# lasseufpa/intent_radio_sched_multi_slice

Hardware: AMD Instinct MI355X
Metric: env-steps/s (batched TTIs) at mult_slice 10-slice/100-UE; 1->8 GPU scaling [device-policy rollout over batch partitions; step-by-step and learner-in-the-loop schedules beside it] (higher is better)
Workload: dtype f64

## Files before the change

### intent_radio_sched_multi_slice_amd/csrc/ranenv_host.cpp

```cpp
#include <algorithm>
#include <cctype>
#include <cmath>
#include <cstdarg>
#include <cstdio>
#include <cstdlib>
#include <cstring>
#include <functional>
#include <new>
#include <string>
#include <array>
#include <vector>

#include "ranenv_internal.h"

using namespace ranenv_dev;

namespace {
thread_local std::string g_last_error;
constexpr int N_STEP_BUILDS = SB_PERSIST_TINY + 1;

}

enum NetRole { NET_INTER, NET_INTRA, NET_INTER_VALUE, NET_INTRA_VALUE, NET_HEAD_CLIP, NET_HEAD_TANH, NET_HEAD_VALUE, NET_SAC_Q };
enum NetForm { FORM_ONE, FORM_SLICE, FORM_MEMBER };
// ... 35 lines not shown
    bool slice_on = false;
    ranenv_trace trace{}; bool trace_on = false;
    std::vector<int32_t> trace_env, trace_slot;
    int32_t *d_trace = nullptr; int trace_cap = 0;
    std::vector<int32_t> sh_steps; bool sh_valid = false;
    const uint8_t *last_done = nullptr;
    int32_t *d_plist = nullptr, *d_pcount = nullptr; PersistCtl *d_pctl = nullptr; unsigned long long *d_pslots = nullptr;
    int p_nclass = 0, p_cap = 0;
    std::vector<int32_t> pcount_host; bool pclass_dirty = true, pcount_host_stale = true;
    bool pclass_maybe = false;
    int *d_cls_flag = nullptr;
    int *h_perr = nullptr;
    int *d_perr_dev = nullptr;
    int perr_seen = 0;
    int last_rollout_persistent = 0, last_rollout_launches = 0;
    long long last_rollout_lean_ttis = 0;
    uint64_t step_launches[N_STEP_BUILDS][2] = {};
    std::string launch_note;
    int p_wave_slots[2] = {0, 0};
    int n_parts = 1;
    std::vector<hipStream_t> part_stream;
    std::vector<hipEvent_t> part_done, part_in;
    std::vector<int> part_lo;
    hipEvent_t ev_in = nullptr;
    bool prof_on = false;
    std::vector<hipEvent_t> prof_ev;
    size_t prof_used = 0;
    long long prof_ttis = 0;
    long long prof_env_ttis = 0;
    struct NetSlot {
// ... 205 lines not shown
    *ev0 = h->prof_ev[h->prof_used]; *ev1 = h->prof_ev[h->prof_used + 1];
    h->prof_used += 2; h->prof_ttis += n_tti; h->prof_env_ttis += (long long)n * n_tti;
    return hipSuccess;
}

const char *const step_build_names[N_STEP_BUILDS] = {"lean", "small", "gather", "tiny1", "mixed", "packed", "persist", "persist_tiny"};

hipError_t launch_step_counted(ranenv_handle h, const StepLaunch &l, dim3 grid, dim3 block, hipStream_t s, hipEvent_t ev0, hipEvent_t ev1, const KP &kp)
{
    const hipError_t e = launch_step(l, grid, block, s, ev0, ev1, kp);
    const bool known = l.build >= 0 && l.build < N_STEP_BUILDS;
    if (e == hipSuccess) {
        if (known && (l.mode & 3) == MODE_STEP) h->step_launches[l.build][l.many ? 1 : 0]++;
        if (l.members) h->last_rollout_member_lines = 1;
        if ((l.mode & 3) == MODE_STEP && l.many && kp.lean_tail != 0 && kp.n_tti > 1) h->last_rollout_lean_ttis += kp.n_tti - 1;
    } else {
        char buf[160];
        snprintf(buf, sizeof(buf), "step kernel build '%s' (row width %d, mode %d, %s, %s): %s", known ? step_build_names[l.build] : "?", l.np, l.mode,
                 l.many ? "several TTIs" : "one TTI", l.gather ? "gather" : "stream", hipGetErrorString(e));
        h->launch_note = buf;
    }
    return e;
}

struct StepFacts { int mode, n_tti, compact; bool gather; int e0, n; bool lines = false, masked = false, tiles = false; };
struct StepChoice { StepLaunch l; dim3 grid, block; int compact; };
StepChoice step_choice(const ranenv *h, const StepFacts &f)
{
    const bool step = f.mode == MODE_STEP;
    const bool pe = f.mode != MODE_RESET && scale_per_element(h);
    const bool many = step && f.n_tti > 1;
    const bool mixed = step && !pe && h->mix != 0 && f.compact != 0 && h->nt == 2 * WAVE && f.e0 == 0 && f.n == h->cfg.batch && !f.masked &&
                       (h->mix == 2 || !persist_tiny(h)) && RANENV_DIAG == 0;
    const int compact = f.compact != 0 && (mixed || f.gather || f.compact == 2) ? 1 : 0;
    const dim3 grid((unsigned)f.n), block((unsigned)h->nt);
    if (mixed) return {{h->np, SB_MIXED, MODE_STEP, many, f.gather}, grid, dim3(2 * WAVE), compact};
    if (step && !pe && h->pack && h->np == 8 && h->cfg.n_ues <= 32 && h->nt == WAVE && (f.n & 1) == 0 && !f.masked && pack_fits_32(h))
        return {{8, SB_PACKED, MODE_STEP, many, f.gather}, dim3((unsigned)(f.n / 2)), dim3(WAVE), compact};
    StepLaunch l{h->np, SB_LEAN, pe ? f.mode | MODE_PE : f.mode, many, f.gather};
    if (f.gather) l.build = SB_GATHER;
    else if (!pe && step && !many && h->tiny_step && persist_tiny(h)) l.build = SB_TINY1;
    else if (!pe && h->small_batch) l.build = SB_SMALL;
    l.members = l.build == SB_LEAN && many && !pe && f.lines && compact != 0 && !f.tiles;
    return {l, grid, block, compact};
}
StepLaunch persist_choice(const ranenv *h, bool lines, bool plain = false)
{
    const bool gather = h->se_mode == RANENV_SE_GATHER, tiny = !gather && !plain && persist_tiny(h);
// ... 489 lines not shown
    {"small_batch", true, [](H h, long long v) { h->small_batch = v != 0; return 0; }, [](H h) -> long long { return h->small_batch ? 1 : 0; }},
    {"tiny_step", true, [](H h, long long v) { h->tiny_step = v != 0 ? 1 : 0; return 0; }, [](H h) -> long long { return h->tiny_step; }},
    {"persist", true, [](H h, long long v) { h->persist = v < 0 ? -1 : (v != 0 ? 1 : 0); return 0; }, [](H h) -> long long { return h->persist; }},
    {"persist_chunk", true, [](H h, long long v) { h->persist_chunk = v < 1 ? 1 : (v > 1000 ? 1000 : (int)v); return 0; },
     [](H h) -> long long { return h->persist_chunk; }},
    {"persist_grid", true, [](H h, long long v) { h->persist_grid = v < 0 ? 0 : (int)v; return 0; }, [](H h) -> long long { return h->persist_grid; }},
    {"pack", true, [](H h, long long v) { h->pack = v != 0; return 0; }, [](H h) -> long long { return h->pack ? 1 : 0; }},
    {"mix", true, [](H h, long long v) { h->mix = v < 0 ? 0 : (v > 2 ? 2 : (int)v); h->pclass_dirty = true; return 0; },
     [](H h) -> long long { return h->mix; }},
    {"persist_inject_abort", false, [](H h, long long v) { h->persist_inject = v != 0 ? 1 : 0; return 0; }, nullptr},
    {"collect_split", true, [](H h, long long v) { h->collect_split = v < 0 ? -1 : (v != 0 ? 1 : 0); return 0; }, [](H h) -> long long { return h->collect_split; }},
    {"autoreset_shortcut", true, [](H h, long long v) { h->autoreset_shortcut = v != 0 ? 1 : 0; return 0; },
     [](H h) -> long long { return h->autoreset_shortcut; }},
    {"member_lines", true, [](H h, long long v) { h->member_lines = v < 0 ? -1 : (v != 0 ? 1 : 0); return 0; }, [](H h) -> long long { return h->member_lines; }},
    {"lean_tail", true, [](H h, long long v) { h->kp.lean_tail = v != 0 ? 1 : 0; return 0; }, [](H h) -> long long { return h->kp.lean_tail; }},
};

const Option *find_option(const std::string &k)
{
    for (const Option &o : options) if (k == o.key) return &o;
    return nullptr;
}

int fuse_first_index(const std::string &k)
{
    return k.rfind("fuse_first", 0) == 0 && k.size() == 11 && k[10] >= '0' && k[10] <= '9' ? k[10] - '0' : -1;
}

int set_option(ranenv_handle h, const std::string &k, long long v)
{
// ... 64 lines not shown
    if (cfg->device < 0 || cfg->device >= ndev) return fail(nullptr, RANENV_E_INVALID, "device %d out of range (%d)", cfg->device, ndev);
    ranenv_handle h = new (std::nothrow) ranenv();
    if (!h) return fail(nullptr, RANENV_E_NOMEM, "out of host memory");
    h->cfg = *cfg;
    HIP_TRY(h, hipSetDevice(cfg->device));
    const size_t B = (size_t)cfg->batch, NS = (size_t)cfg->n_scenarios, D = (size_t)cfg->hist_depth;
    const size_t L = (size_t)cfg->max_age_cap + 1;
    KP &kp = h->kp;
    memset(&kp, 0, sizeof(kp));
    kp.B = cfg->batch; kp.S = S; kp.U = U; kp.R = R; kp.G = cfg->rbs_per_rbg; kp.Us = Us; kp.D = cfg->hist_depth;
    kp.L = (int)L; kp.max_steps = cfg->max_steps; kp.flags = cfg->flags; kp.T = R / cfg->rbs_per_rbg;
    kp.policy = RANENV_POLICY_MARR; kp.fixed_intra = RANENV_INTRA_RR;
    kp.bw_hz = cfg->bandwidth_hz; kp.bw_per_rb = cfg->bandwidth_hz / (double)R; kp.over = cfg->overfulfill;
    kp.norm_traffic = cfg->norm_traffic; kp.norm_ues = cfg->norm_ues; kp.norm_se = cfg->norm_se;
    kp.lean_tail = 1;
    int rc = RANENV_OK;
#define ALLOC(field, count) if (rc == RANENV_OK) rc = dev_alloc(h, &field, (count))
    const size_t NSL = (size_t)S * GRP;
    kp.BU = (long long)(B * U); kp.NSU = (long long)(NS * U); kp.NSL = (long long)(NS * NSL);
    ALLOC(kp.tab.slice_i32, NS * S * 8); ALLOC(kp.tab.slice_f64, NS * S * 2);
    ALLOC(kp.tab.param_i32, 2 * NS * S * 6); ALLOC(kp.tab.param_f64, 2 * NS * S * 3);
    ALLOC(kp.tab.slice_ues, NS * S * Us); ALLOC(kp.tab.slice_usecase, NS * S);
    ALLOC(kp.tab.ue, (size_t)N_TUE * NS * U); ALLOC(kp.tab.slot, 3 * NS * NSL);
    ALLOC(kp.st.u4, (size_t)N_U4 * B * U); ALLOC(kp.st.u8, (size_t)N_U8 * B * U); ALLOC(kp.st.b4, (size_t)N_B4 * B);
    ALLOC(kp.st.age_ring, B * L * U); ALLOC(kp.st.ring_sent, B * D * U); ALLOC(kp.st.ring_drop, B * D * U);
    ALLOC(kp.st.mask_inter, B * S); ALLOC(kp.st.mask_intra, B * S * Us); ALLOC(kp.st.policy_scores, B * S);
    ALLOC(h->d_episodes, B); ALLOC(h->d_ar_mask, B); ALLOC(h->d_members, NS); ALLOC(h->d_cls_flag, 1);
#undef ALLOC
    if (rc != RANENV_OK) { std::string m = h->err; ranenv_destroy(h); g_last_error = m; return rc; }
    kp.episodes = h->d_episodes;
// ... 44 lines not shown
            HIP_TRY(h, hipSetDevice(h->cfg.device)); HIP_TRY(h, hipDeviceSynchronize());
            std::vector<PersistCtl> ctl((size_t)h->p_nclass);
            HIP_TRY(h, hipMemcpy(ctl.data(), h->d_pctl, sizeof(PersistCtl) * ctl.size(), hipMemcpyDeviceToHost));
            for (auto &c : ctl) for (int x = 0; x < 8; x++) tot += (long long)c.stat[x][which];
        }
        *value = tot;
    }
    else if (k == "persist_errors") {
        int v = 0;
        if (h->h_perr) { HIP_TRY(h, hipSetDevice(h->cfg.device)); HIP_TRY(h, hipDeviceSynchronize()); v = *(volatile int *)h->h_perr != 0 ? 1 : 0; }
        *value = h->perr_seen + v;
    }
    else if (k == "last_rollout_persistent") *value = h->last_rollout_persistent;
    else if (k == "last_rollout_launches") *value = h->last_rollout_launches;
    else if (k == "last_rollout_member_lines") *value = h->last_rollout_member_lines;
    else if (k == "last_rollout_lean_ttis") *value = h->last_rollout_lean_ttis;
    else if (k.rfind("step_launches_", 0) == 0) {
        std::string b = k.substr(14);
        const bool many_only = b.size() > 5 && b.compare(b.size() - 5, 5, "_many") == 0;
        if (many_only) b.resize(b.size() - 5);
        int which = -1;
        for (int i = 0; i < N_STEP_BUILDS; i++) if (b == step_build_names[i]) which = i;
        if (which < 0) return fail(h, RANENV_E_INVALID, "unknown option '%s'", key);
        *value = (int64_t)(h->step_launches[which][1] + (many_only ? 0 : h->step_launches[which][0]));
    }
    else if (const int i = fuse_first_index(k); i >= 0) *value = (size_t)i < h->fuse_first.size() ? h->fuse_first[(size_t)i] : 0;
    else return fail(h, RANENV_E_INVALID, "unknown option '%s'", key);
    return RANENV_OK;
}

// ... 2176 lines not shown
}

struct RolloutPlan { bool persistent; int fuse; bool member_lines; };
constexpr long long PERSIST_GATHER_MAX_ENVS_PER_CU = 44, PERSIST_STREAM_MAX_ENVS_PER_CU = 20, PERSIST_STREAM_MIN_TTIS = 4, PERSIST_STREAM_MAX_TTIS = 64;
constexpr int PERSIST_MAX_EPISODE_ENDS = 2;
constexpr int FUSE_ROLLOUT_PART = 4, FUSE_MAX_TTIS = 10;
static RolloutPlan rollout_plan(const ranenv *h, const Rollout &r, bool capturing)
{
    const int k = r.n_steps;
    const long long B = h->cfg.batch, N = h->n_cus;
    const bool gather = h->se_mode == RANENV_SE_GATHER;
    const bool one_tti = r.kp.head_obs || r.kp.head_reward || r.net || slice_metrics_on(h) || trace_on(h);
    RolloutPlan p{false, one_tti ? 1 : (h->fuse > 0 ? h->fuse : std::clamp(k / FUSE_ROLLOUT_PART, 1, FUSE_MAX_TTIS)), false};
    const bool wins = persist_tiny(h) || (!h->small_batch && (gather ? B <= PERSIST_GATHER_MAX_ENVS_PER_CU * N
                          : B <= PERSIST_STREAM_MAX_ENVS_PER_CU * N && k >= PERSIST_STREAM_MIN_TTIS && k <= PERSIST_STREAM_MAX_TTIS));
    p.persistent = (RANENV_DIAG == 0 || RANENV_DIAG == 12) && (h->persist == 1 || (h->persist < 0 && wins)) && !one_tti && !scale_per_element(h) &&
                   r.kp.compact != 0 && (B >> PERSIST_ENV_BITS) == 0 && !capturing;
    int n_ends = 0;
    if (p.persistent && h->persist < 0 && r.follow) (void)ttis_to_end(h, r, 0, h->cfg.batch, k, &n_ends);
    p.persistent = p.persistent && n_ends <= PERSIST_MAX_EPISODE_ENDS;
    const StepFacts chunk{MODE_STEP, 2, r.kp.compact, gather, 0, h->n_parts > 1 ? h->part_lo[1] : h->cfg.batch, true};
    p.member_lines = h->member_lines != 0 && h->kp.se_pool != nullptr &&
                     (p.persistent ? persist_choice(h, true).members : k > 1 && p.fuse > 1 && step_choice(h, chunk).l.members);
    return p;
}

static int rollout_chunks(ranenv_handle h, Rollout &r, int fuse, hipStream_t stream)
{
    const int n_steps = r.n_steps;
    const int np = h->n_parts > 1 ? h->n_parts : 1;
    std::vector<int> pdone((size_t)np, 0), pn((size_t)np, 0);
// ... 38 lines not shown
    rc = slice_metrics_outputs(h, obs_intra, reward);
    if (rc != RANENV_OK) return rc;
    rc = trace_outputs(h, nullptr, obs_inter, obs_intra, reward, done);
    if (rc != RANENV_OK) return rc;
    if (h->kp.policy == RANENV_POLICY_EXTERNAL) return fail(h, RANENV_E_STATE, "a rollout needs a device policy (ranenv_set_policy MARR / MAPF / NETWORK)");
    if (head_inter(h) && h->head.on && !obs_inter) return fail(h, RANENV_E_INVALID, "the policy network reads obs_inter: the step needs that buffer");
    const bool have_se = h->kp.se_pool != nullptr || (h->se_mode == RANENV_SE_GATHER && h->d_se_mean != nullptr);
    if (!have_se || (!h->kp.trf_pool && !h->kp.trf_gen)) return fail(h, RANENV_E_STATE, "a rollout replays the bound SE pool and traffic pool / generator");
    HIP_TRY(h, hipSetDevice(h->cfg.device));
    rc = persist_check_errors(h);
    if (rc != RANENV_OK) return rc;
    hipStream_t stream = (hipStream_t)stream_;
    Rollout r;
    r.n_steps = n_steps;
    r.kp = call_kp(h, obs_inter, obs_intra, reward, done);
    h->last_rollout_persistent = 0; h->last_rollout_launches = 0; h->last_rollout_member_lines = 0; h->last_rollout_lean_ttis = 0;
    r.net = net_use(h, r.kp);
    if (r.net < 0) return r.net;
    r.rec = rec;
    rc = compact_for(h, r.kp, stream, &r.kp.compact);
    if (rc != RANENV_OK) return rc;
    if (r.kp.compact) r.kp.compact = 2;
    r.follow = h->ar_on;
    if (r.follow) {
        if (!done) return fail(h, RANENV_E_INVALID, "a rollout with auto-reset needs the done buffer");
        std::vector<int32_t> &steps = r.steps;
        steps.resize((size_t)h->cfg.batch);
        HIP_TRY(h, hipStreamSynchronize(stream));
        HIP_TRY(h, hipMemcpy(steps.data(), ST_step_no(h->kp), sizeof(int32_t) * steps.size(), hipMemcpyDeviceToHost));
        r.adv = advance_args(h, done, obs_inter, obs_intra, nullptr, nullptr, nullptr);
        r.kpr = reset_behind(h, r.kp);
// ... 794 lines not shown
```

### intent_radio_sched_multi_slice_amd/csrc/ranenv_internal.h

```cpp
#pragma once
#include <hip/hip_runtime.h>
#include <hip/hip_ext.h>

#include <cstddef>
#include <cstdint>

#include "ranenv.h"

#ifndef RANENV_DIAG
#define RANENV_DIAG 0
#endif

namespace ranenv_dev {

enum { MODE_STEP = 0, MODE_DENSE = 1, MODE_RESET = 2,
       MODE_PE = 4 };

struct Tables {
    int32_t *slice_i32;
    double  *slice_f64;
    int32_t *param_i32;
    double  *param_f64;
    int32_t *slice_ues;
    int32_t *slot;
    int32_t *slice_usecase;
// ... 66 lines not shown
struct KP {
    int B, S, U, R, G, Us, D, L, max_steps, flags, policy, fixed_intra;
    long long BU, NSU, NSL;
    int T;
    int e0;
    int n_tti;
    int compact;
    double bw_hz, bw_per_rb, over, norm_traffic, norm_ues, norm_se;
    Tables tab;
    State st;
    const ranenv_episode *episodes;
    const float *se_pool; long long se_stride;
    int se_quad;
    const double *se_mean_pool;
    int se_rp;
    const int32_t *trf_pool;
    int trf_gen; int env_id_base; unsigned long long trf_seed;
    const unsigned long long *pois_cdf;
    const uint8_t *pois_guide;
    const int32_t *max_steps_env;
    double *acc;
    const uint8_t *env_mask;
    const double *scores; const uint8_t *intra; const double *traffic_bits; const float *se_tiles;
    const uint8_t *dense;
    float *obs_inter; float *obs_intra; double *reward; uint8_t *done;
    float *head_obs; double *head_reward;
    const int32_t *p_list;
    int p_count, p_chunk;
    const int32_t *m_list;
    const int32_t *m_counts;
    struct PersistCtl *p_ctl;
    unsigned long long *p_slots;
    int p_cap;
    int lean_tail;
    int *p_err;
    const float *ml_pool; long long ml_stride;
};
static_assert(offsetof(KP, p_err) - offsetof(KP, lean_tail) == 4 && offsetof(KP, lean_tail) - offsetof(KP, p_cap) == 4, "KP: lean_tail fills the padding behind p_cap");

constexpr int WAVE = 64;
constexpr int GRP = 16;

struct AdvanceArgs {
    const uint8_t *done; uint8_t *mask;
    ranenv_episode *episodes; const ranenv_episode *table; int table_first, table_n;
    int32_t *episode_no, *reset_count;
    int initial, max_ep, random, env_id_base; unsigned long long seed;
    const float *obs_inter, *obs_intra, *head_obs; float *term_inter, *term_intra, *term_head;
    int n_inter, n_intra, n_head;
    int e0;
    int *cls_flag;
    const double *acc; double *ep_acc; int32_t *ep_n; int ep_slots;
    const double *head_acc; double *head_ep_acc;
// ... 264 lines not shown
```

### intent_radio_sched_multi_slice_amd/csrc/ranenv_step_body.hpp

```cpp
#pragma once
#include "ranenv_numeric.hpp"

namespace {

#if RANENV_DIAG == 9
#define RANENV_STAMP(k) do { if (!PERSIST && threadIdx.x == 0 && (k) < p.S) \
    ST_policy_scores(p)[(size_t)(p.e0 + blockIdx.x) * p.S + (k)] = (double)__builtin_amdgcn_s_memrealtime(); } while (0)
#elif RANENV_DIAG == 12
#define RANENV_STAMP(k) do { if constexpr (PERSIST) if (tid == 0) { const unsigned long long now_ = __builtin_amdgcn_s_memrealtime(); \
    double *d_ = &ST_policy_scores(p)[(size_t)e * p.S]; \
    if ((k) == 0) { if (warm) acc_add(d_, (double)(now_ - cy.last_stamp)); acc_add(d_ + 9, 1.0); } else acc_add(d_ + (k), (double)(now_ - stamp_prev)); \
    stamp_prev = now_; if ((k) == 8) cy.last_stamp = now_; } } while (0)
#else
#define RANENV_STAMP(k) do { } while (0)
#endif


template <int NP>
struct SharedCore {
    double rows[NP][4 * NP + 2];
    double xr[4][GRP];
    double pf[NP][3];
    double sf[NP][2];
    int si[NP][8];
// ... 247 lines not shown
    long long win_sent;
    double sem_prev;
    long long sum_age, win_drop;
    int front, front_rem, fifo;
    int pf_old_s, pf_old_d, pf_traffic;
    int2 pf1, pf2;
#if RANENV_DIAG == 12
    unsigned long long last_stamp;
#endif
};

struct NoMemberLines { };
template <int MODE_X, int NQ, bool GATHER, int NP, bool PERSIST = false, int PACK = 1, bool MIX = false, bool MEMBERS = false, bool LEAN = false, typename P>
DEVFN bool step_body(const P &p, StepCarry &cy, const bool warm, const int e_in,
                     std::conditional_t<PACK == 2, SeStreamLane<GATHER ? 1 : NQ>, SeStream<GATHER ? 1 : NQ>> *se_carry = nullptr,
                     const bool se_ready = false, const bool se_next = false, const bool narrow_in = false, const bool tail_in = true)
{
    constexpr int MODE = MODE_X & 3;
    constexpr bool PE = (MODE_X & MODE_PE) != 0;
    static_assert(!PE || (MODE != MODE_RESET && !PERSIST && PACK == 1 && !MIX), "per-element scaling: the lean step / dense builds");
    static_assert(!(GATHER && MODE == MODE_DENSE), "a dense sched_decision reads whole rows: streaming only");
    static_assert(!MEMBERS || (MODE == MODE_STEP && !PE && !GATHER && PACK == 1 && !MIX && NQ < 8), "member lines: the lean step builds of rollouts");
    static_assert(PACK == 1 || (PACK == 2 && MODE == MODE_STEP && !PERSIST), "packed waves: step launches only");
    static_assert(!LEAN || MODE == MODE_STEP, "a launch of several TTIs steps");
    constexpr int LW = WAVE / PACK;
    constexpr int GDEPTH = (GATHER && NQ == 0) ? 1 : 2;
    constexpr bool CARRY = PERSIST && MODE == MODE_STEP && PACK == 1 && !GATHER && NQ >= 8;
    static_assert(!MIX || (PACK == 1 && MODE == MODE_STEP), "mixed blocks: step launches, one env per wave or per block");
    const bool narrow = MIX && narrow_in;
    __shared__ SharedCore<NP> shs[MIX ? 2 : PACK];
    int e_ = PACK == 2 ? e_in + (int)(threadIdx.x >> 5) : __builtin_amdgcn_readfirstlane(e_in);
// ... 16 lines not shown
#if RANENV_DIAG == 12
    unsigned long long stamp_prev = 0;
#endif
    RANENV_STAMP(0);
    typedef const __attribute__((address_space(4))) KP *kp_const_t;
    kp_const_t kc = (kp_const_t)__builtin_amdgcn_kernarg_segment_ptr();
    asm volatile("" : "+s"(kc));
#define COLD(f) (kc->f)
    bool tail_v = true, rows_v = true;
    if constexpr (LEAN) {
        tail_v = __builtin_amdgcn_readfirstlane(tail_in ? 1 : 0) != 0;
        rows_v = tail_v || COLD(acc) != nullptr;
    }
#define TAIL (!LEAN || tail_v)
#define ROWS (!LEAN || rows_v)
    ranenv_episode ep;
    int t, hlen, npush, se_pos, trf_pos;
    if (!warm) {
        ep = p.episodes[e];
        ep.scenario = uni(ep.scenario); ep.se_offset = uni(ep.se_offset); ep.trf_offset = uni(ep.trf_offset);
        ep.se_len = uni(ep.se_len); ep.trf_len = uni(ep.trf_len);
        ep.se_base = uni64(ep.se_base); ep.trf_base = uni64(ep.trf_base);
        t = (MODE == MODE_RESET) ? 0 : uni(ST_step_no(p)[e]);
        hlen = uni(ST_hist_len(p)[e]);
        npush = uni(ST_n_push(p)[e]);
        se_pos = (MODE == MODE_RESET) ? ep.se_offset : uni(ST_se_pos(p)[e]);
        trf_pos = (MODE == MODE_RESET) ? ep.trf_offset : uni(ST_trf_pos(p)[e]);
    } else {
        ep.scenario = uni(cy.ep.scenario); ep.se_offset = uni(cy.ep.se_offset); ep.trf_offset = uni(cy.ep.trf_offset);
        ep.se_len = uni(cy.ep.se_len); ep.trf_len = uni(cy.ep.trf_len); ep.reserved = 0;
// ... 23 lines not shown
    const unsigned lane4 = (unsigned)lane * 4u;
#define TBL(f) row_at<PACK>(TB_##f(p), tb_row, lane4)
    int u, slc, ue_pos, pkt_size, max_pkts, max_age;
    if (!warm) {
        u = compact ? TBL(lane_ue) : lane;
        slc = TBL(ue_slice); ue_pos = TBL(ue_pos);
        pkt_size = TBL(ue_pkt_size); max_pkts = TBL(ue_max_pkts); max_age = TBL(ue_max_age);
    } else {
        u = cy.u; slc = cy.slc; ue_pos = cy.ue_pos; pkt_size = cy.pkt_size; max_pkts = cy.max_pkts; max_age = cy.max_age;
        asm volatile("" : "+v"(u), "+v"(slc), "+v"(ue_pos));
    }
#undef TBL
    const bool act = tid < U && !(compact && slc < 0);
    if (!PERSIST && PACK == 1 && !warm && compact && __builtin_amdgcn_ballot_w64(act) == 0 && tid >= WAVE) return true;
    const size_t er4 = (size_t)e * U * 4, er8 = (size_t)e * U * 8;
    const unsigned u4 = (unsigned)u * 4u, u8 = (unsigned)u * 8u;
#define UE4(f) row_at<PACK>(ST_##f(p), er4, u4)
#define UE8(f) row_at<PACK>(ST_##f(p), er8, u8)
    const int ptot = uni(warm ? cy.ptot : ST_push_total(p)[e]);
    const int cmark = uni(warm ? cy.cmark : ST_clear_mark(p)[e]);
    int lastp = ptot;
    int total = 0, front = 0, front_rem = 0, fifo = 0, rb_start = 0, rb_count = 0;
    long long sum_age = 0, win_sent = 0, win_drop = 0;
    double sem_prev = 0.0;
    if (warm) { total = cy.total; win_sent = cy.win_sent; sem_prev = cy.sem_prev; }
    else {
        if (MODE != MODE_RESET) total = UE4(queue_pkts);
        if (!clear_hist) win_sent = UE8(win_sent);
    }
    auto ring_s = [&]() { return &row_at<PACK>(ST_ring_sent(p), ((size_t)e * D + npush) * U * 4, u4); };
    auto ring_d = [&]() { return &row_at<PACK>(ST_ring_drop(p), ((size_t)e * D + npush) * U * 4, u4); };
    int old_s = 0, old_d = 0;
    double traffic = 0.0;
    const bool gen_traffic = MODE != MODE_RESET && p.traffic_bits == nullptr && p.trf_gen != 0;
    const bool carried = CARRY && warm;
    auto rest_of_state = [&]() {
        if (carried) {
            sum_age = cy.sum_age; front = cy.front; front_rem = cy.front_rem; fifo = cy.fifo; win_drop = cy.win_drop;
            old_s = cy.pf_old_s; old_d = cy.pf_old_d;
            if (!gen_traffic) traffic = (double)cy.pf_traffic;
            return;
        }
        if (MODE != MODE_RESET) {
            sum_age = UE8(queue_age_sum);
            front = UE4(front); front_rem = UE4(front_rem); fifo = UE4(fifo);
        }
        if (!clear_hist) { win_drop = UE8(win_dropped); lastp = UE4(last_push); }
        if (hlen == D) { old_s = *ring_s(); old_d = *ring_d(); }
        if (MODE != MODE_RESET && !gen_traffic)
            traffic = p.traffic_bits ? row_at<PACK>(p.traffic_bits, er8, u8)
                                     : (double)row_at<PACK>(p.trf_pool, PACK == 2 ? (size_t)trf_row32 : ((size_t)ep.trf_base + (size_t)trf_pos) * U * 4, u4);
    };
    constexpr bool STATE_AT_ENTRY = !GATHER && NQ >= 8;
    if constexpr (STATE_AT_ENTRY) rest_of_state();
    if (MODE == MODE_STEP && !warm) sem_prev = UE8(se_mean);
    double sem_tile = 0.0;
    if (GATHER) sem_tile = row_at<PACK>(p.se_mean_pool, (size_t)tile_no * U * 8, u8);
    int st_si0 = 0, st_si1 = 0, st_pi0 = 0, st_pi1 = 0; double st_pf = 0.0, st_sf = 0.0;
    if (tid < WAVE && !warm) {
        const unsigned t4 = (unsigned)tid * 4u, t8 = (unsigned)tid * 8u;
        if (tid < S * 8) st_si0 = row_at<PACK>(TB_slice_i32(p), (size_t)sc * S * 32, t4);
        if (tid + LW < S * 8) st_si1 = row_at<PACK>(TB_slice_i32(p), (size_t)sc * S * 32, t4 + LW * 4u);
// ... 62 lines not shown
            if constexpr (PACK == 1) {
                unsigned short *desc = reinterpret_cast<unsigned short *>(&sh.xr[0][0]) + (narrow ? 0 : (tid >> 6)) * 64;
                spread = gather_part_spread<PE>(tile, U * p.se_rp * 4, u * p.se_rp * 4, R, (unsigned)rb_start, (unsigned)rb_count, PE ? COLD(bw_per_rb) : 1.0, desc, my_part);
            }
            if (!spread) my_part = gather_part<PACK, GDEPTH, PE>(tile, U * p.se_rp * 4, u * p.se_rp * 4, R, (unsigned)rb_start, (unsigned)rb_count, PE ? COLD(bw_per_rb) : 1.0);
        }
    } else if constexpr (MODE == MODE_STEP) {
        const unsigned us1 = (unsigned)rb_start, uc1 = (unsigned)rb_count;
        if constexpr (MEMBERS) member_line_sums(ml, R, us1, uc1, hook);
        else row_sums<PE>(se1, R, [=](int r) { return ((unsigned)r - us1) < uc1; }, my_full, my_part, hook, PE ? COLD(bw_per_rb) : 1.0);
    } else if constexpr (MODE == MODE_DENSE) {
        const uint8_t *mrow = p.dense + ((size_t)e * U + u) * R;
        row_sums<PE>(se1, R, [=](int r) { return mrow[r] != 0; }, my_full, my_part, hook, PE ? COLD(bw_per_rb) : 1.0);
    } else {
        row_sums(se1, R, [](int) { return false; }, my_full, my_part, hook);
    }
    if constexpr (!STATE_AT_ENTRY) rest_of_state();
    if constexpr (MEMBERS) member_line_finish(ml, R, (unsigned)rb_start, (unsigned)rb_count, my_full, my_part);
    if constexpr (SE_AHEAD && CARRY) {
        if (se_next) {
            const int pos_next = se_pos + 1 >= ep.se_len ? 0 : se_pos + 1;
            asm volatile("" ::: "memory");
            se1.init(p.se_pool + (size_t)(ep.se_base + (long long)pos_next) * (size_t)p.se_stride, U, u, R, se_quad);
            asm volatile("" ::: "memory");
        }
    }
    RANENV_STAMP(3);
    wg_sync(narrow);
    RANENV_STAMP(4);

// ... 72 lines not shown
                int slot = npush - (ptot - q); slot += slot < 0 ? D : 0;
                const unsigned so = (unsigned)(slot * U + u) * 4u;
                int32_t *qs = &row_at<PACK>(ST_ring_sent(p), (size_t)e * D * U * 4, so), *qd = &row_at<PACK>(ST_ring_drop(p), (size_t)e * D * U * 4, so);
                if (q - cmark >= D) { win_sent -= *qs; win_drop -= *qd; }
                *qs = 0; *qd = 0;
            }
        }
        if (MODE == MODE_RESET && clear_hist) {
            for (int k = 0; k < D; k++) {
                row_at<PACK>(ST_ring_sent(p), ((size_t)e * D + k) * U * 4, u4) = 0;
                row_at<PACK>(ST_ring_drop(p), ((size_t)e * D + k) * U * 4, u4) = 0;
            }
        }
        win_sent += sent - old_s; win_drop += dropped - old_d;
        nt_store<GATHER>(*ring_s(), (int32_t)sent); nt_store<GATHER>(*ring_d(), (int32_t)dropped);
        UE4(last_push) = ptot + 1;
        UE4(queue_pkts) = total; UE8(queue_age_sum) = sum_age;
        UE4(front) = front; UE4(front_rem) = front_rem; UE4(fifo) = fifo;
        UE8(win_sent) = win_sent; UE8(win_dropped) = win_drop;
        if (TAIL) {
            UE4(pkt_effective_thr) = (int32_t)sent; UE4(dropped_pkts) = (int32_t)dropped;
            if (!(COLD(flags) & RANENV_F_NO_RAW_OUTPUT)) {
                nt_store<GATHER>(UE4(pkt_incoming), (int32_t)pkt_in); nt_store<GATHER>(UE4(pkt_throughputs), (int32_t)pkt_thr);
            }
        }
        sent_u = sent; drop_u = dropped;

        UE8(se_mean) = se_mean_new; sem_new = se_mean_new;
        UE4(rb_start) = rb_start; UE4(rb_count) = rb_count;
        if constexpr (CARRY) {
            cy.sum_age = sum_age; cy.win_drop = win_drop; cy.front = front; cy.front_rem = front_rem; cy.fifo = fifo;
            int ps = 0, pd = 0, pt = 0;
            int2 e1 = make_int2(0, 0), e2 = make_int2(0, 0);
            if (se_next) {
                const int np1 = npush + 1 == D ? 0 : npush + 1;
                if (hlen_new == D) {
                    if (D == 1) { ps = sent; pd = dropped; }
                    else {
                        ps = row_at<PACK>(ST_ring_sent(p), ((size_t)e * D + np1) * U * 4, u4);
                        pd = row_at<PACK>(ST_ring_drop(p), ((size_t)e * D + np1) * U * 4, u4);
                    }
                }
                if (!gen_traffic) {
                    const int tp1 = trf_pos + 1 >= ep.trf_len ? 0 : trf_pos + 1;
// ... 247 lines not shown
    RANENV_STAMP(7);

    RANENV_STAMP(8);
    if (MODE == MODE_STEP) {
        cy.ep = ep; cy.t = t + 1; cy.hlen = hlen_new; cy.npush = npush + 1 == D ? 0 : npush + 1;
        cy.se_pos = se_pos + 1 >= ep.se_len ? 0 : se_pos + 1; cy.trf_pos = trf_pos + 1 >= ep.trf_len ? 0 : trf_pos + 1;
        cy.ptot = ptot + 1; cy.cmark = (ptot + 1 - cmark > 2 * D) ? ptot + 1 - 2 * D : cmark; cy.episode_no = episode_no;
        cy.u = u; cy.slc = slc; cy.ue_pos = ue_pos; cy.pkt_size = pkt_size; cy.max_pkts = max_pkts; cy.max_age = max_age;
        cy.total = total; cy.win_sent = win_sent; cy.sem_prev = act ? sem_new : sem_prev;
    }
    return false;
#undef UE4
#undef UE8
#undef TAIL
#undef ROWS
}

template <int MODE_X, int NQ, bool GATHER, int NP, bool MANY, int PACK = 1, bool MIX = false, bool MEMBERS = false>
DEVFN void step_loop(const KP &p)
{
    constexpr int MODE = MODE_X & 3;
    if constexpr (MODE == MODE_STEP) {
        bool narrow = false;
        int e_mix = 0;
        if constexpr (MIX) {
            const int b = (int)blockIdx.x, n_wide = p.m_counts[1], n_narrow = p.m_counts[0];
            const int k8 = b & 7;
            if (b < n_wide) {
                const int q_ = n_wide >> 3, r_ = n_wide & 7;
                e_mix = p.p_list[k8 * q_ + (k8 < r_ ? k8 : r_) + (b >> 3)];
// ... 8 lines not shown
                const int idx = 2 * pos + __builtin_amdgcn_readfirstlane((int)(threadIdx.x >> 6));
                if (idx >= n_narrow) return;
                e_mix = p.m_list[idx];
            }
        }
        typedef const __attribute__((address_space(4))) KP *kp_const_t;
        const int n = MANY ? (p.n_tti < 1 ? 1 : p.n_tti) : 1;
        StepCarry cy = {};
        bool warm = false;
        for (int k = 0; k < n; k++) {
            kp_const_t kc = (kp_const_t)__builtin_amdgcn_kernarg_segment_ptr();
            asm volatile("" : "+s"(kc));
            const int nb_ = (int)gridDim.x, xk_ = (int)blockIdx.x & 7, q_ = nb_ >> 3, r_ = nb_ & 7;
            const int b_perm = xk_ * q_ + (xk_ < r_ ? xk_ : r_) + ((int)blockIdx.x >> 3);
            const bool tail = !MANY || k + 1 == n || kc->lean_tail == 0;
            if (step_body<MODE_X, NQ, GATHER, NP, false, PACK, MIX, MEMBERS, MANY>(*kc, cy, warm, MIX ? e_mix : kc->e0 + b_perm * PACK, nullptr, false, false, narrow, tail)) return;
            if (k + 1 < n) {
                warm = MANY;
                if (warm) wg_sync(narrow); else full_sync(narrow);
            }
        }
    } else {
        StepCarry cy = {};
        step_body<MODE_X, NQ, GATHER, NP>(p, cy, false, p.e0 + (int)blockIdx.x);
    }
}
#undef COLD

struct PersistLocal { int item, next, keep, fresh_mask, xcc, pad; };
enum { PERSIST_EXIT = -1, PERSIST_NONE = -2 };

// ... 122 lines not shown
        int done = (int)((unsigned)item >> PERSIST_ENV_BITS);
        StepCarry cy = {};
        SeStream<GATHER ? 1 : NQ> seq;
        bool warm = false, se_ready = false;
        for (;;) {
            kp_const_t kc0 = (kp_const_t)__builtin_amdgcn_kernarg_segment_ptr();
            asm volatile("" : "+s"(kc0));
            const int n_tti = kc0->n_tti, left = n_tti - done;
            int want = kc0->p_chunk;
            if (done == 0 && want > 1 && want < n_tti) want = 1 + (int)((((unsigned)e * 0x9E3779B1u) >> 16) % (unsigned)want);
            const int n = left < want ? left : want;
            for (int k = 0; k < n; k++) {
                kp_const_t kc = (kp_const_t)__builtin_amdgcn_kernarg_segment_ptr();
                asm volatile("" : "+s"(kc));
                const bool ahead = done + k + 1 < n_tti;
                (void)step_body<MODE_STEP, NQ, GATHER, NP, true, 1, false, MEMBERS, true>(*kc, cy, warm, e, &seq, se_ready, ahead, false, !ahead || kc->lean_tail == 0);
                se_ready = ahead;
                if (k + 1 < n) { warm = true; wg_sync(); }
            }
            done += n;
            full_sync();
            if (tid0 == 0) {
                kp_const_t kc = (kp_const_t)__builtin_amdgcn_kernarg_segment_ptr();
                asm volatile("" : "+s"(kc));
                pl.keep = persist_finish(*kc, pl, e, done, n_tti);
            }
            __syncthreads();
            if (uni(pl.keep) == 0) break;
            warm = true;
        }
    }
}

#ifndef RANENV_CLASS_PRIO
#define RANENV_CLASS_PRIO 1
#endif
#define RANENV_PERSIST_WPE ((NP == 16) ? 4 : 5)
template <bool GATHER, int NP>
__global__ void __launch_bounds__(CORE_NT) __attribute__((amdgpu_waves_per_eu(RANENV_PERSIST_WPE, RANENV_PERSIST_WPE))) ranenv_persist_kernel(const KP p)
{
    (void)p;
#if RANENV_DIAG == 0 || RANENV_DIAG == 12
#if RANENV_CLASS_PRIO
    if ((blockDim.x == WAVE) == GATHER) __builtin_amdgcn_s_setprio(RANENV_CLASS_PRIO);
#endif
    persist_loop<GATHER ? 1 : SE_DEPTH_LEAN, GATHER, NP>();
#endif
}

template <int NP>
__global__ void __launch_bounds__(CORE_NT) __attribute__((amdgpu_waves_per_eu(RANENV_PERSIST_WPE, RANENV_PERSIST_WPE))) ranenv_persist_kernel_members(const KP p)
{
    (void)p;
#if RANENV_DIAG == 0 || RANENV_DIAG == 12
#if RANENV_CLASS_PRIO
    if (blockDim.x != WAVE) __builtin_amdgcn_s_setprio(RANENV_CLASS_PRIO);
#endif
    persist_loop<SE_DEPTH_LEAN, false, NP, true>();
#endif
}

template <int NP>
__global__ void __launch_bounds__(CORE_NT) __attribute__((amdgpu_waves_per_eu(2, 2))) ranenv_persist_kernel_tiny(const KP p)
{
    (void)p;
#if RANENV_DIAG == 0 || RANENV_DIAG == 12
    persist_loop<SE_DEPTH_TINY, false, NP>();
#endif
}

template <int NP>
__global__ void __launch_bounds__(CORE_NT) __attribute__((amdgpu_waves_per_eu(2, 2))) ranenv_core_kernel_tiny1(const KP p)
{
    step_loop<MODE_STEP, SE_DEPTH_TINY, false, NP, false>(p);
}
#define RANENV_CORE_ATTR __attribute__((amdgpu_waves_per_eu(5, 5)))
template <int MODE, int NP, bool MANY>
__global__ void __launch_bounds__(CORE_NT) RANENV_CORE_ATTR ranenv_core_kernel(const KP p)
{
    step_loop<MODE, ((MODE & 3) == MODE_DENSE || NP == 16) ? 1 : SE_DEPTH_LEAN, false, NP, MANY>(p);
}
// ... 29 lines not shown
```

Before: 115.3 million.

## Keep per-UE queue state in registers across fused TTIs, flush at chunk end

Result: faster. 123.4 million, median of 6 (+7.0%).

```diff
diff --git a/intent_radio_sched_multi_slice_amd/csrc/ranenv_host.cpp b/intent_radio_sched_multi_slice_amd/csrc/ranenv_host.cpp
--- a/intent_radio_sched_multi_slice_amd/csrc/ranenv_host.cpp
+++ b/intent_radio_sched_multi_slice_amd/csrc/ranenv_host.cpp
@@ -73,6 +73,7 @@
     int *d_perr_dev = nullptr;
     int perr_seen = 0;
     int last_rollout_persistent = 0, last_rollout_launches = 0;
+    long long last_rollout_kept_state_ttis = 0;
     long long last_rollout_lean_ttis = 0;
     uint64_t step_launches[N_STEP_BUILDS][2] = {};
     std::string launch_note;
@@ -308,6 +309,7 @@
         if (known && (l.mode & 3) == MODE_STEP) h->step_launches[l.build][l.many ? 1 : 0]++;
         if (l.members) h->last_rollout_member_lines = 1;
         if ((l.mode & 3) == MODE_STEP && l.many && kp.lean_tail != 0 && kp.n_tti > 1) h->last_rollout_lean_ttis += kp.n_tti - 1;
+        if ((l.mode & 3) == MODE_STEP && l.many && kp.lean_state != 0 && kp.n_tti > 1) h->last_rollout_kept_state_ttis += kp.n_tti - 1;
     } else {
         char buf[160];
         snprintf(buf, sizeof(buf), "step kernel build '%s' (row width %d, mode %d, %s, %s): %s", known ? step_build_names[l.build] : "?", l.np, l.mode,
@@ -325,7 +327,7 @@
     const bool pe = f.mode != MODE_RESET && scale_per_element(h);
     const bool many = step && f.n_tti > 1;
     const bool mixed = step && !pe && h->mix != 0 && f.compact != 0 && h->nt == 2 * WAVE && f.e0 == 0 && f.n == h->cfg.batch && !f.masked &&
-                       (h->mix == 2 || !persist_tiny(h)) && RANENV_DIAG == 0;
+                       (h->mix == 2 || !persist_tiny(h)) && (RANENV_DIAG == 0 || RANENV_DIAG == 13);
     const int compact = f.compact != 0 && (mixed || f.gather || f.compact == 2) ? 1 : 0;
     const dim3 grid((unsigned)f.n), block((unsigned)h->nt);
     if (mixed) return {{h->np, SB_MIXED, MODE_STEP, many, f.gather}, grid, dim3(2 * WAVE), compact};
@@ -845,6 +847,7 @@
      [](H h) -> long long { return h->autoreset_shortcut; }},
     {"member_lines", true, [](H h, long long v) { h->member_lines = v < 0 ? -1 : (v != 0 ? 1 : 0); return 0; }, [](H h) -> long long { return h->member_lines; }},
     {"lean_tail", true, [](H h, long long v) { h->kp.lean_tail = v != 0 ? 1 : 0; return 0; }, [](H h) -> long long { return h->kp.lean_tail; }},
+    {"lean_state", true, [](H h, long long v) { h->kp.lean_state = v != 0 ? 1 : 0; return 0; }, [](H h) -> long long { return h->kp.lean_state; }},
 };
 
 const Option *find_option(const std::string &k)
@@ -939,6 +942,7 @@
     kp.bw_hz = cfg->bandwidth_hz; kp.bw_per_rb = cfg->bandwidth_hz / (double)R; kp.over = cfg->overfulfill;
     kp.norm_traffic = cfg->norm_traffic; kp.norm_ues = cfg->norm_ues; kp.norm_se = cfg->norm_se;
     kp.lean_tail = 1;
+    kp.lean_state = 1;
     int rc = RANENV_OK;
 #define ALLOC(field, count) if (rc == RANENV_OK) rc = dev_alloc(h, &field, (count))
     const size_t NSL = (size_t)S * GRP;
@@ -1013,6 +1017,7 @@
     else if (k == "last_rollout_persistent") *value = h->last_rollout_persistent;
     else if (k == "last_rollout_launches") *value = h->last_rollout_launches;
     else if (k == "last_rollout_member_lines") *value = h->last_rollout_member_lines;
+    else if (k == "last_rollout_kept_state_ttis") *value = h->last_rollout_kept_state_ttis;
     else if (k == "last_rollout_lean_ttis") *value = h->last_rollout_lean_ttis;
     else if (k.rfind("step_launches_", 0) == 0) {
         std::string b = k.substr(14);
@@ -3219,7 +3224,7 @@
     RolloutPlan p{false, one_tti ? 1 : (h->fuse > 0 ? h->fuse : std::clamp(k / FUSE_ROLLOUT_PART, 1, FUSE_MAX_TTIS)), false};
     const bool wins = persist_tiny(h) || (!h->small_batch && (gather ? B <= PERSIST_GATHER_MAX_ENVS_PER_CU * N
                           : B <= PERSIST_STREAM_MAX_ENVS_PER_CU * N && k >= PERSIST_STREAM_MIN_TTIS && k <= PERSIST_STREAM_MAX_TTIS));
-    p.persistent = (RANENV_DIAG == 0 || RANENV_DIAG == 12) && (h->persist == 1 || (h->persist < 0 && wins)) && !one_tti && !scale_per_element(h) &&
+    p.persistent = (RANENV_DIAG == 0 || RANENV_DIAG == 12 || RANENV_DIAG == 13) && (h->persist == 1 || (h->persist < 0 && wins)) && !one_tti && !scale_per_element(h) &&
                    r.kp.compact != 0 && (B >> PERSIST_ENV_BITS) == 0 && !capturing;
     int n_ends = 0;
     if (p.persistent && h->persist < 0 && r.follow) (void)ttis_to_end(h, r, 0, h->cfg.batch, k, &n_ends);
@@ -3288,7 +3293,7 @@
     Rollout r;
     r.n_steps = n_steps;
     r.kp = call_kp(h, obs_inter, obs_intra, reward, done);
-    h->last_rollout_persistent = 0; h->last_rollout_launches = 0; h->last_rollout_member_lines = 0; h->last_rollout_lean_ttis = 0;
+    h->last_rollout_persistent = 0; h->last_rollout_launches = 0; h->last_rollout_member_lines = 0; h->last_rollout_lean_ttis = 0; h->last_rollout_kept_state_ttis = 0;
     r.net = net_use(h, r.kp);
     if (r.net < 0) return r.net;
     r.rec = rec;
diff --git a/intent_radio_sched_multi_slice_amd/csrc/ranenv_internal.h b/intent_radio_sched_multi_slice_amd/csrc/ranenv_internal.h
--- a/intent_radio_sched_multi_slice_amd/csrc/ranenv_internal.h
+++ b/intent_radio_sched_multi_slice_amd/csrc/ranenv_internal.h
@@ -9,6 +9,9 @@
 
 #ifndef RANENV_DIAG
 #define RANENV_DIAG 0
+#endif
+#ifndef RANENV_KEEP_STATE
+#define RANENV_KEEP_STATE 1
 #endif
 
 namespace ranenv_dev {
@@ -105,6 +108,7 @@
     int se_quad;
     const double *se_mean_pool;
     int se_rp;
+    int lean_state;
     const int32_t *trf_pool;
     int trf_gen; int env_id_base; unsigned long long trf_seed;
     const unsigned long long *pois_cdf;
@@ -128,6 +132,7 @@
     const float *ml_pool; long long ml_stride;
 };
 static_assert(offsetof(KP, p_err) - offsetof(KP, lean_tail) == 4 && offsetof(KP, lean_tail) - offsetof(KP, p_cap) == 4, "KP: lean_tail fills the padding behind p_cap");
+static_assert(offsetof(KP, trf_pool) - offsetof(KP, lean_state) == 4 && offsetof(KP, lean_state) - offsetof(KP, se_rp) == 4, "KP: lean_state fills the padding behind se_rp");
 
 constexpr int WAVE = 64;
 constexpr int GRP = 16;
diff --git a/intent_radio_sched_multi_slice_amd/csrc/ranenv_step_body.hpp b/intent_radio_sched_multi_slice_amd/csrc/ranenv_step_body.hpp
--- a/intent_radio_sched_multi_slice_amd/csrc/ranenv_step_body.hpp
+++ b/intent_radio_sched_multi_slice_amd/csrc/ranenv_step_body.hpp
@@ -285,7 +285,8 @@
 template <int MODE_X, int NQ, bool GATHER, int NP, bool PERSIST = false, int PACK = 1, bool MIX = false, bool MEMBERS = false, bool LEAN = false, typename P>
 DEVFN bool step_body(const P &p, StepCarry &cy, const bool warm, const int e_in,
                      std::conditional_t<PACK == 2, SeStreamLane<GATHER ? 1 : NQ>, SeStream<GATHER ? 1 : NQ>> *se_carry = nullptr,
-                     const bool se_ready = false, const bool se_next = false, const bool narrow_in = false, const bool tail_in = true)
+                     const bool se_ready = false, const bool se_next = false, const bool narrow_in = false, const bool tail_in = true,
+                     const bool flush_in = true)
 {
     constexpr int MODE = MODE_X & 3;
     constexpr bool PE = (MODE_X & MODE_PE) != 0;
@@ -332,6 +333,14 @@
     }
 #define TAIL (!LEAN || tail_v)
 #define ROWS (!LEAN || rows_v)
+    constexpr bool KEEPS = LEAN && RANENV_DIAG != 13 && (CARRY || (PACK == 1 && RANENV_KEEP_STATE != 0));
+    bool flush_v = true, keep_v = false;
+    if constexpr (LEAN) {
+        const bool on = COLD(lean_state) != 0;
+        flush_v = __builtin_amdgcn_readfirstlane(flush_in ? 1 : 0) != 0 || !on;
+        keep_v = warm && on;
+    }
+#define FLUSH (!LEAN || flush_v)
     ranenv_episode ep;
     int t, hlen, npush, se_pos, trf_pos;
     if (!warm) {
@@ -385,7 +394,10 @@
     const bool act = tid < U && !(compact && slc < 0);
     if (!PERSIST && PACK == 1 && !warm && compact && __builtin_amdgcn_ballot_w64(act) == 0 && tid >= WAVE) return true;
     const size_t er4 = (size_t)e * U * 4, er8 = (size_t)e * U * 8;
-    const unsigned u4 = (unsigned)u * 4u, u8 = (unsigned)u * 8u;
+    unsigned u4 = (unsigned)u * 4u, u8 = (unsigned)u * 8u;
+    constexpr bool WHO = KEEPS && !CARRY;
+    [[maybe_unused]] unsigned who = 0;
+    if constexpr (WHO) who = (unsigned)u | ((unsigned)(slc + 1) << 16) | ((unsigned)ue_pos << 24);
 #define UE4(f) row_at<PACK>(ST_##f(p), er4, u4)
 #define UE8(f) row_at<PACK>(ST_##f(p), er8, u8)
     const int ptot = uni(warm ? cy.ptot : ST_push_total(p)[e]);
@@ -412,11 +424,26 @@
             if (!gen_traffic) traffic = (double)cy.pf_traffic;
             return;
         }
+        if constexpr (LEAN) {
+#if RANENV_DIAG == 13
+            const bool kept = keep_v;
+#else
+            const bool kept = KEEPS && keep_v;
+            if constexpr (KEEPS) if (kept) { sum_age = cy.sum_age; front = cy.front; front_rem = cy.front_rem; fifo = cy.fifo; win_drop = cy.win_drop; }
+#endif
+            if (!kept) {
+                sum_age = UE8(queue_age_sum);
+                front = UE4(front); front_rem = UE4(front_rem); fifo = UE4(fifo);
+                win_drop = UE8(win_dropped);
+            }
+            if (!keep_v) lastp = UE4(last_push);
+        } else {
         if (MODE != MODE_RESET) {
             sum_age = UE8(queue_age_sum);
             front = UE4(front); front_rem = UE4(front_rem); fifo = UE4(fifo);
         }
         if (!clear_hist) { win_drop = UE8(win_dropped); lastp = UE4(last_push); }
+        }
         if (hlen == D) { old_s = *ring_s(); old_d = *ring_d(); }
         if (MODE != MODE_RESET && !gen_traffic)
             traffic = p.traffic_bits ? row_at<PACK>(p.traffic_bits, er8, u8)
@@ -509,6 +536,11 @@
         row_sums<PE>(se1, R, [=](int r) { return mrow[r] != 0; }, my_full, my_part, hook, PE ? COLD(bw_per_rb) : 1.0);
     } else {
         row_sums(se1, R, [](int) { return false; }, my_full, my_part, hook);
+    }
+    if constexpr (WHO) {
+        asm volatile("" : "+v"(who));
+        u = (int)(who & 0xffffu); slc = (int)((who >> 16) & 0xffu) - 1; ue_pos = (int)(who >> 24);
+        u4 = (unsigned)u * 4u; u8 = (unsigned)u * 8u;
     }
     if constexpr (!STATE_AT_ENTRY) rest_of_state();
     if constexpr (MEMBERS) member_line_finish(ml, R, (unsigned)rb_start, (unsigned)rb_count, my_full, my_part);
@@ -611,10 +643,20 @@
         }
         win_sent += sent - old_s; win_drop += dropped - old_d;
         nt_store<GATHER>(*ring_s(), (int32_t)sent); nt_store<GATHER>(*ring_d(), (int32_t)dropped);
+        if constexpr (LEAN) {
+            if (FLUSH) {
+                UE4(last_push) = ptot + 1; UE4(queue_pkts) = total; UE8(win_sent) = win_sent;
+                UE8(se_mean) = se_mean_new; UE4(rb_start) = rb_start; UE4(rb_count) = rb_count;
+            }
+            if (FLUSH || !(KEEPS || RANENV_DIAG == 13)) {
+                UE8(queue_age_sum) = sum_age; UE4(front) = front; UE4(front_rem) = front_rem; UE4(fifo) = fifo; UE8(win_dropped) = win_drop;
+            }
+        } else {
         UE4(last_push) = ptot + 1;
         UE4(queue_pkts) = total; UE8(queue_age_sum) = sum_age;
         UE4(front) = front; UE4(front_rem) = front_rem; UE4(fifo) = fifo;
         UE8(win_sent) = win_sent; UE8(win_dropped) = win_drop;
+        }
         if (TAIL) {
             UE4(pkt_effective_thr) = (int32_t)sent; UE4(dropped_pkts) = (int32_t)dropped;
             if (!(COLD(flags) & RANENV_F_NO_RAW_OUTPUT)) {
@@ -623,8 +665,9 @@
         }
         sent_u = sent; drop_u = dropped;
 
-        UE8(se_mean) = se_mean_new; sem_new = se_mean_new;
-        UE4(rb_start) = rb_start; UE4(rb_count) = rb_count;
+        sem_new = se_mean_new;
+        if constexpr (!LEAN) { UE8(se_mean) = se_mean_new; UE4(rb_start) = rb_start; UE4(rb_count) = rb_count; }
+        if constexpr (KEEPS && !CARRY) { cy.sum_age = sum_age; cy.win_drop = win_drop; cy.front = front; cy.front_rem = front_rem; cy.fifo = fifo; }
         if constexpr (CARRY) {
             cy.sum_age = sum_age; cy.win_drop = win_drop; cy.front = front; cy.front_rem = front_rem; cy.fifo = fifo;
             int ps = 0, pd = 0, pt = 0;
@@ -902,6 +945,7 @@
 #undef UE8
 #undef TAIL
 #undef ROWS
+#undef FLUSH
 }
 
 template <int MODE_X, int NQ, bool GATHER, int NP, bool MANY, int PACK = 1, bool MIX = false, bool MEMBERS = false>
@@ -940,7 +984,8 @@
             const int nb_ = (int)gridDim.x, xk_ = (int)blockIdx.x & 7, q_ = nb_ >> 3, r_ = nb_ & 7;
             const int b_perm = xk_ * q_ + (xk_ < r_ ? xk_ : r_) + ((int)blockIdx.x >> 3);
             const bool tail = !MANY || k + 1 == n || kc->lean_tail == 0;
-            if (step_body<MODE_X, NQ, GATHER, NP, false, PACK, MIX, MEMBERS, MANY>(*kc, cy, warm, MIX ? e_mix : kc->e0 + b_perm * PACK, nullptr, false, false, narrow, tail)) return;
+            const bool flush = !MANY || k + 1 == n;
+            if (step_body<MODE_X, NQ, GATHER, NP, false, PACK, MIX, MEMBERS, MANY>(*kc, cy, warm, MIX ? e_mix : kc->e0 + b_perm * PACK, nullptr, false, false, narrow, tail, flush)) return;
             if (k + 1 < n) {
                 warm = MANY;
                 if (warm) wg_sync(narrow); else full_sync(narrow);
@@ -1093,7 +1138,8 @@
                 kp_const_t kc = (kp_const_t)__builtin_amdgcn_kernarg_segment_ptr();
                 asm volatile("" : "+s"(kc));
                 const bool ahead = done + k + 1 < n_tti;
-                (void)step_body<MODE_STEP, NQ, GATHER, NP, true, 1, false, MEMBERS, true>(*kc, cy, warm, e, &seq, se_ready, ahead, false, !ahead || kc->lean_tail == 0);
+                const bool flush = k + 1 == n || !ahead;
+                (void)step_body<MODE_STEP, NQ, GATHER, NP, true, 1, false, MEMBERS, true>(*kc, cy, warm, e, &seq, se_ready, ahead, false, !ahead || kc->lean_tail == 0, flush);
                 se_ready = ahead;
                 if (k + 1 < n) { warm = true; wg_sync(); }
             }
@@ -1119,7 +1165,7 @@
 __global__ void __launch_bounds__(CORE_NT) __attribute__((amdgpu_waves_per_eu(RANENV_PERSIST_WPE, RANENV_PERSIST_WPE))) ranenv_persist_kernel(const KP p)
 {
     (void)p;
-#if RANENV_DIAG == 0 || RANENV_DIAG == 12
+#if RANENV_DIAG == 0 || RANENV_DIAG == 12 || RANENV_DIAG == 13
 #if RANENV_CLASS_PRIO
     if ((blockDim.x == WAVE) == GATHER) __builtin_amdgcn_s_setprio(RANENV_CLASS_PRIO);
 #endif
@@ -1131,7 +1177,7 @@
 __global__ void __launch_bounds__(CORE_NT) __attribute__((amdgpu_waves_per_eu(RANENV_PERSIST_WPE, RANENV_PERSIST_WPE))) ranenv_persist_kernel_members(const KP p)
 {
     (void)p;
-#if RANENV_DIAG == 0 || RANENV_DIAG == 12
+#if RANENV_DIAG == 0 || RANENV_DIAG == 12 || RANENV_DIAG == 13
 #if RANENV_CLASS_PRIO
     if (blockDim.x != WAVE) __builtin_amdgcn_s_setprio(RANENV_CLASS_PRIO);
 #endif
@@ -1143,7 +1189,7 @@
 __global__ void __launch_bounds__(CORE_NT) __attribute__((amdgpu_waves_per_eu(2, 2))) ranenv_persist_kernel_tiny(const KP p)
 {
     (void)p;
-#if RANENV_DIAG == 0 || RANENV_DIAG == 12
+#if RANENV_DIAG == 0 || RANENV_DIAG == 12 || RANENV_DIAG == 13
     persist_loop<SE_DEPTH_TINY, false, NP>();
 #endif
 }
```
